# toposware/certificate-stark

Measured on NVIDIA B200. Metric: state_transition_prove_throughput, higher is better.
Workload: dtype u64 (f63 modular)

## Files before the change

### certificate_stark_b200/csrc/airs.cuh

```cuda
#pragma once
#include "ecc.cuh"
#include "rescue.cuh"
#include "rescue_tables.h"
#include <stdexcept>

#if defined(__CUDA_ARCH__)
#define CSG_PRAGMA_(x) _Pragma(#x)
#define CSG_PRAGMA(x) CSG_PRAGMA_(x)
#else
#define CSG_PRAGMA(x)
#endif
#ifndef CSG_REST_UNROLL
#define CSG_REST_UNROLL 1
#endif
#if defined(__CUDA_ARCH__)
#define CSG_REST_LOOP CSG_PRAGMA(unroll CSG_REST_UNROLL)
#else
#define CSG_REST_LOOP
#endif
#ifndef CSG_RESCUE_FWD_UNROLL
#define CSG_RESCUE_FWD_UNROLL 2
#endif

namespace airs {
using f63::fe;

enum : int { TRANSACTION = 0, MERKLE_UPDATE = 1, MERKLE_INIT = 2, SCHNORR = 3, RANGE = 4, RESCUE = 5 };

enum : int {
    HSW = 14, HRW = 7, APW = 12, PPW = 18, PCW = 6,
    SENDER_INITIAL = 0, SENDER_BIT = 14, SENDER_UPDATED = 15, RECEIVER_INITIAL = 29, RECEIVER_BIT = 43, RECEIVER_UPDATED = 44,
    PREV_ROOT = 58, VALUE_RES = 65, BALANCE_RES = 90, NONCE_RES = 91, INT_ROOT_RES = 92, ROOT_MATCH_RES = 99,
    SENDER_KEY = 65, RECEIVER_KEY = 77, DELTA_COPY = 89, SIGMA_COPY = 90, NONCE_COPY = 91,
    SENDER_KEY_RES = 101, RECEIVER_KEY_RES = 103, DELTA_COPY_RES = 105, SIGMA_COPY_RES = 106, NONCE_COPY_RES = 107,
    DELTA_RANGE_RES = 108, SIGMA_RANGE_RES = 109,
    DELTA_BIT = 56, DELTA_ACC = 57, SIGMA_BIT = 92, SIGMA_ACC = 93,
    LIMBS = 2 * PPW + 1,
    SIG_HASH = 2 * PPW + 6
};
enum : int {
    TX_SETUP = 0, TX_MERKLE = 1, TX_HASH_INPUT = 2, TX_FINISH = 3, TX_HASH = 4, TX_SCHNORR = 5, TX_SCALAR_MULT = 6, TX_DOUBLING = 7,
    TX_DIGEST = 8, TX_SCHNORR_HASH = 12, TX_INTERNAL = 13, TX_RANGE_STEP = 17, TX_RANGE_FINISH = 18, TX_VALUE_COPY = 19, TX_ARK = 20
};

constexpr int MAX_GROUPS = 8;

struct Frame {
    const fe *cur_p, *next_p;
    size_t stride;
    CSG_HD fe cur(int c) const { return cur_p[(size_t)c * stride]; }
    CSG_HD fe next(int c) const { return next_p[(size_t)c * stride]; }
};
struct Periodic {
    const fe *tab;
    const uint32_t *off, *mask;
    uint32_t i;
    CSG_HD fe operator()(int c) const { return tab[off[c] + (i & mask[c])]; }
};

#if defined(__CUDACC__)
static __host__ __device__ __noinline__
#else
inline
#endif
fe slot_coefficient(const fe *alpha, const fe *beta, const uint8_t *group, const fe *xp, size_t xp_stride, int slot) {
    return f63::add(alpha[slot], f63::mul(beta[slot], xp[group[slot] * xp_stride]));
}

constexpr int MAX_SPLIT_GROUPS = 6;
template <bool SPLIT, int DEG = 1>
struct CombT {
    static constexpr bool split = SPLIT;
    static constexpr int D = DEG;

    const fe *alpha, *beta;
    const uint8_t *group;
    const fe *xp;
    size_t xp_stride;
// ... 95 lines not shown

CSG_HD fe f_not(fe a) { return f63::sub(f63::ONE, a); }
CSG_HD fe f_bin(fe a) { return f63::sub(f63::sqr(a), a); }

template <class PV, class CB>
CSG_HD void rescue_state(const Frame &f, const PV &pv, CB &C, int col0, int ark0, fe flag_a, int slot_a, bool second, fe flag_b, int slot_b) {
    fe tc[14], tn[14];
#if defined(__CUDA_ARCH__)
#pragma unroll
#endif
    for (int j = 0; j < 14; j++) {
        tc[j] = rescue::cube(f.cur(col0 + j));
        tn[j] = f63::sub(f.next(col0 + j), pv(ark0 + 14 + j));
    }
    FlagAcc a(flag_a), b(flag_b);
#if defined(__CUDA_ARCH__)
#pragma unroll 1
#endif
    for (int i = 0; i < 14; i++) {
        const uint64_t *mds = CSG_TABLE(CSG_MDS) + i * 14, *inv_mds = CSG_TABLE(CSG_INV_MDS) + i * 14;
        f63::acc128 fwd, bwd;
#if defined(__CUDA_ARCH__)
#pragma unroll
#endif
        for (int j = 0; j < 14; j++) { fwd.mac(mds[j], tc[j]); bwd.mac(inv_mds[j], tn[j]); }
        const fe d = f63::sub(rescue::cube(bwd.reduce()), f63::add(fwd.reduce(), pv(ark0 + i)));
        a.add(C, slot_a + i, d);
        if (second) b.add(C, slot_b + i, d);
    }
    a.flush(C);
    if (second) b.flush(C);
}

template <class CB>
CSG_HD void merkle_auth_path(const Frame &f, CB &C, int base, fe tx_hash, fe hash_input, fe hashf) {
    const fe copy_flag = f63::mul(tx_hash, f_not(f63::add(hashf, hash_input)));
    const fe init_flag = f63::mul(tx_hash, hash_input);
    const fe bit = f.next(base + HSW), nbit = f_not(bit);
    C.add(base + HSW, f63::mul(tx_hash, f_bin(bit)));
    const fe init_bit = f63::mul(init_flag, bit), init_nbit = f63::mul(init_flag, nbit);
    FlagAcc keep(f63::add(copy_flag, init_nbit)), to_rate(init_bit), place_bit(init_bit), place_nbit(init_nbit);
#if defined(__CUDA_ARCH__)
#pragma unroll 1
#endif
    for (int k = 0; k < 2; k++) {
        const int o = base + k * (HSW + 1);
        CSG_REST_LOOP
        for (int i = 0; i < HRW; i++) {
            fe c = f.cur(o + i);
            keep.add(C, o + i, f63::sub(c, f.next(o + i)));
            to_rate.add(C, o + HRW + i, f63::sub(c, f.next(o + HRW + i)));
        }
        C.sync();
    }
    CSG_REST_LOOP
    for (int i = 0; i < HRW; i++) place_bit.add(C, base + i, f63::sub(f.next(base + HSW + 1 + i), f.next(base + i)));
    CSG_REST_LOOP
    for (int i = HRW; i < HSW; i++) place_nbit.add(C, base + i, f63::sub(f.next(base + HSW + 1 + i), f.next(base + i)));
    C.sync();
    keep.flush(C);
    to_rate.flush(C);
    place_bit.flush(C);
    place_nbit.flush(C);
}
template <class CB>
CSG_HD void merkle_roots(const Frame &f, CB &C, fe finish) {
    FlagAcc carry(f_not(finish)), fin(finish);
    CSG_REST_LOOP
    for (int i = 0; i < HRW; i++) {
        fe nr = f.next(PREV_ROOT + i), cr = f.cur(PREV_ROOT + i);
        carry.add(C, PREV_ROOT + i, f63::sub(nr, cr));
        fin.add(C, PREV_ROOT + i, f63::sub(nr, f.next(RECEIVER_UPDATED + i)));
        fin.add(C, INT_ROOT_RES + i, f63::sub(f.cur(SENDER_UPDATED + i), f.cur(RECEIVER_INITIAL + i)));
        fin.add(C, ROOT_MATCH_RES + i, f63::sub(f.next(SENDER_INITIAL + i), cr));
    }
    carry.flush(C);
    fin.flush(C);
}
template <class CB>
CSG_HD void value_block(const Frame &f, CB &C, FlagAcc &a) {
    CSG_REST_LOOP
    for (int i = 0; i < APW; i++) {
        a.add(C, VALUE_RES + i, f63::sub(f.cur(SENDER_INITIAL + i), f.cur(SENDER_UPDATED + i)));
        a.add(C, VALUE_RES + APW + i, f63::sub(f.cur(RECEIVER_INITIAL + i), f.cur(RECEIVER_UPDATED + i)));
    }
    a.add(C, VALUE_RES + 2 * APW, f63::sub(f.cur(RECEIVER_INITIAL + APW + 1), f.cur(RECEIVER_UPDATED + APW + 1)));
    a.add(C, BALANCE_RES, f63::sub(f63::sub(f.cur(SENDER_INITIAL + APW), f.cur(SENDER_UPDATED + APW)),
                                   f63::sub(f.cur(RECEIVER_UPDATED + APW), f.cur(RECEIVER_INITIAL + APW))));
    a.add(C, NONCE_RES, f63::sub(f.cur(SENDER_UPDATED + APW + 1), f63::add(f.cur(SENDER_INITIAL + APW + 1), f63::ONE)));
}

template <class CB>
CSG_HD void scalar_mult_bank(const Frame &f, CB &C, int o, const fe (&q)[12], fe doubling, fe addition) {
    auto load_point = [&]() {
        ecc::point p;
#if defined(__CUDA_ARCH__)
#pragma unroll
#endif
        for (int i = 0; i < 6; i++) { p.x.c[i] = f.cur(o + i); p.y.c[i] = f.cur(o + 6 + i); p.z.c[i] = f.cur(o + 12 + i); }
        return p;
    };
    const fe bit = f.cur(o + PPW);
    {
        ecc::point d = ecc::double_point(load_point());
        FlagAcc a(doubling);
        for (int i = 0; i < 6; i++) {
            a.add(C, o + i, f63::sub(f.next(o + i), d.x.c[i]));
            a.add(C, o + 6 + i, f63::sub(f.next(o + 6 + i), d.y.c[i]));
            a.add(C, o + 12 + i, f63::sub(f.next(o + 12 + i), d.z.c[i]));
        }
        a.add(C, o + PPW, f_bin(bit));
        a.flush(C);
    }
// ... 8 lines not shown
        }
        a.add(C, o + PPW, f63::sub(bit, f.next(o + PPW)));
        a.flush(C);
    }
}
template <class CB>
CSG_HD void scalar_mult_bank_outputs(const Frame &f, CB &C, int o, const fe (&q)[12], int formula) {
    ecc::point p;
#if defined(__CUDA_ARCH__)
#pragma unroll
#endif
    for (int i = 0; i < 6; i++) { p.x.c[i] = f.cur(o + i); p.y.c[i] = f.cur(o + 6 + i); p.z.c[i] = f.cur(o + 12 + i); }
    const ecc::point r = formula == 0 ? ecc::double_point(p) : ecc::add_mixed(p, ecc::load6(q), ecc::load6(q + 6));
    FlagAcc a(f63::ONE);
    for (int i = 0; i < 6; i++) a.add(C, o + i, r.x.c[i]);
    for (int i = 0; i < 6; i++) a.add(C, o + 6 + i, r.y.c[i]);
    for (int i = 0; i < 6; i++) a.add(C, o + 12 + i, r.z.c[i]);
    a.flush(C);
}
template <class CB>
CSG_HD fe scalar_mult_bank_merge(const Frame &f, const CB &C, int comp, int o, fe doubling, fe addition, fe Cd, fe Cm) {
    const fe bit = f.cur(o + PPW), nbit = f_not(bit);
    f63::acc192 sd, sa;
    for (int i = 0; i < PPW; i++) {
        const fe c = comp ? C.coef_x(comp, o + i) : C.coef(o + i), nx = f.next(o + i);
        sd.mac(c, nx);
        sa.mac(c, f63::sub(nx, f63::mul(nbit, f.cur(o + i))));
    }
    const fe cb = comp ? C.coef_x(comp, o + PPW) : C.coef(o + PPW);
    const fe td = f63::sub(f63::add(sd.reduce(), f63::mul(cb, f_bin(bit))), Cd);
    const fe ta = f63::sub(f63::add(sa.reduce(), f63::mul(cb, f63::sub(bit, f.next(o + PPW)))), f63::mul(bit, Cm));
    return f63::add(f63::mul(doubling, td), f63::mul(addition, ta));
}
template <class CB>
CSG_HD void schnorr_final_addition(const Frame &f, CB &C, fe final_add) {
    ecc::point s, hp;
    for (int i = 0; i < 6; i++) {
        s.x.c[i] = f.cur(i); s.y.c[i] = f.cur(6 + i); s.z.c[i] = f.cur(12 + i);
        hp.x.c[i] = f.cur(PPW + 1 + i); hp.y.c[i] = f.cur(PPW + 7 + i); hp.z.c[i] = f.cur(PPW + 13 + i);
    }
    ecc::point r = ecc::add_full(s, hp);
    ecc::fp6 nx;
    for (int i = 0; i < 6; i++) nx.c[i] = f.next(i);
    ecc::fp6 xz = ecc::mul(nx, r.z);
    FlagAcc a(final_add);
    for (int i = 0; i < 6; i++) {
        a.add(C, i, f63::sub(xz.c[i], r.x.c[i]));
        a.add(C, 6 + i, f63::sub(f.next(6 + i), r.y.c[i]));
        a.add(C, 12 + i, f63::sub(f.next(12 + i), r.z.c[i]));
    }
    for (int i = 0; i < 4; i++) a.add(C, LIMBS + 1 + i, f63::sub(f.cur(LIMBS + 1 + i), f.cur(SIG_HASH + i)));
    a.flush(C);
}
template <class IN, class CB>
CSG_HD void schnorr_light(const Frame &f, CB &C, fe doubling, fe addition, const fe (&digest)[4], fe copy_hash, IN in) {
    const fe hbit_next = f.next(LIMBS);
    FlagAcc hold(addition);
    CSG_REST_LOOP
    for (int i = 0; i < 4; i++) {
        const int c = LIMBS + 4 - i;
        fe cv = f.cur(c), nv = f.next(c);
        C.add(c, f63::mul(f63::mul(digest[i], doubling), f63::sub(nv, f63::add(f63::dbl(cv), hbit_next))));
        C.add(c, f63::mul(f63::mul(f_not(digest[i]), doubling), f63::sub(cv, nv)));
        hold.add(C, LIMBS + 1 + i, f63::sub(f.cur(LIMBS + 1 + i), f.next(LIMBS + 1 + i)));
    }
    hold.flush(C);
    C.sync();
    FlagAcc a(copy_hash);
    CSG_REST_LOOP
    for (int i = 0; i < HRW; i++) {
        a.add(C, SIG_HASH + i, f63::sub(f.cur(SIG_HASH + i), f.next(SIG_HASH + i)));
        a.add(C, SIG_HASH + HRW + i, f63::sub(f.next(SIG_HASH + HRW + i), in(i)));
    }
    a.flush(C);
}

template <int AIR> struct Items;
template <> struct Items<TRANSACTION> { static constexpr int rescue = 5, ecc = 3; };
template <> struct Items<MERKLE_UPDATE> { static constexpr int rescue = 4, ecc = 0; };
template <> struct Items<MERKLE_INIT> { static constexpr int rescue = 4, ecc = 0; };
template <> struct Items<SCHNORR> { static constexpr int rescue = 1, ecc = 3; };
template <> struct Items<RANGE> { static constexpr int rescue = 0, ecc = 0; };
template <> struct Items<RESCUE> { static constexpr int rescue = 1, ecc = 0; };

struct RescueItem { int col0, ark0, slot_a, slot_b; bool second; };
CSG_HD constexpr RescueItem rescue_item(int air, int s) {
    return air == TRANSACTION ? (s < 4 ? RescueItem{15 * s - (s >> 1), TX_ARK, 14 * s, 15 * s - (s >> 1), true} : RescueItem{SIG_HASH, TX_ARK, SIG_HASH, 0, false})
         : air == MERKLE_UPDATE ? RescueItem{15 * s - (s >> 1), 5, 15 * s - (s >> 1), 0, false}
// ... 111 lines not shown
            else if (s == 2) rescue_state_t<rescue_item_ng(TRANSACTION, 2, 0), rescue_item_ng(TRANSACTION, 2, 1)>(f, pv, C, it.col0, it.ark0, flag_a, 4, flag_b, 5);
            else if (s == 3) rescue_state_t<rescue_item_ng(TRANSACTION, 3, 0), rescue_item_ng(TRANSACTION, 3, 1)>(f, pv, C, it.col0, it.ark0, flag_a, 6, flag_b, 7);
            else rescue_state_t<rescue_item_ng(TRANSACTION, 4, 0), 0>(f, pv, C, it.col0, it.ark0, flag_a, 8, 0, 0);
        } else rescue_state_t<1, 0>(f, pv, C, it.col0, it.ark0, flag_a, 2 * s, 0, 0);
        return;
    }
    rescue_state(f, pv, C, it.col0, it.ark0, flag_a, it.slot_a, it.second, flag_b, it.slot_b);
}
template <int AIR, class PV, class CB>
CSG_HD void eval_ecc_bank(int bank, const Frame &f, const PV &pv, CB &C) {
    if (AIR != TRANSACTION && AIR != SCHNORR) return;
    const fe scalar_mult = pv(AIR == TRANSACTION ? TX_SCALAR_MULT : 1);
    const fe doubling = pv(AIR == TRANSACTION ? TX_DOUBLING : 2), addition = f63::mul(f_not(doubling), scalar_mult);
    fe q[12];
    const uint64_t *gen = CSG_TABLE(CSG_GENERATOR);
    for (int j = 0; j < 12; j++) q[j] = bank == 0 ? gen[j] : (AIR == TRANSACTION ? f.next(SENDER_KEY + j) : pv(7 + j));
    scalar_mult_bank(f, C, bank * (PPW + 1), q, doubling, addition);
}
template <int AIR, class PV, class CB>
CSG_HD void eval_ecc_bank_outputs(int bank, int formula, const Frame &f, const PV &pv, CB &C) {
    if (AIR != TRANSACTION && AIR != SCHNORR) return;
    fe q[12];
    const uint64_t *gen = CSG_TABLE(CSG_GENERATOR);
    for (int j = 0; j < 12; j++) q[j] = bank == 0 ? gen[j] : (AIR == TRANSACTION ? f.next(SENDER_KEY + j) : pv(7 + j));
    scalar_mult_bank_outputs(f, C, bank * (PPW + 1), q, formula);
}
template <int AIR, class PV, class CB>
CSG_HD fe eval_ecc_bank_merge(int bank, const Frame &f, const PV &pv, const CB &C, int comp, fe Cd, fe Cm) {
    if (AIR != TRANSACTION && AIR != SCHNORR) return 0;
    const fe scalar_mult = pv(AIR == TRANSACTION ? TX_SCALAR_MULT : 1);
    const fe doubling = pv(AIR == TRANSACTION ? TX_DOUBLING : 2), addition = f63::mul(f_not(doubling), scalar_mult);
    return scalar_mult_bank_merge(f, C, comp, bank * (PPW + 1), doubling, addition, Cd, Cm);
}
template <int AIR, class PV, class CB>
CSG_HD void eval_ecc_final(const Frame &f, const PV &pv, CB &C) {
    if (AIR != TRANSACTION && AIR != SCHNORR) return;
    const fe mask = pv(AIR == TRANSACTION ? TX_SCHNORR : 0), scalar_mult = pv(AIR == TRANSACTION ? TX_SCALAR_MULT : 1);
    schnorr_final_addition(f, C, f63::mul(f_not(scalar_mult), mask));
}

template <class PV, class CB>
CSG_HD void rest_transaction(const Frame &f, const PV &pv, CB &C) {
    const fe setup = pv(TX_SETUP), tx_hash = pv(TX_MERKLE), hash_input = pv(TX_HASH_INPUT), finish = pv(TX_FINISH), hashf = pv(TX_HASH);
    const fe schnorr_mask = pv(TX_SCHNORR), scalar_mult = pv(TX_SCALAR_MULT), doubling = pv(TX_DOUBLING), schnorr_hash = pv(TX_SCHNORR_HASH);
    const fe copy_hash = f63::mul(f_not(schnorr_hash), schnorr_mask);
    const fe addition = f63::mul(f_not(doubling), scalar_mult);
    {
        FlagAcc a(setup);
        value_block(f, C, a);
        C.sync();
        CSG_REST_LOOP
        for (int o = 0; o < APW; o++) {
            a.add(C, SENDER_KEY_RES + o, f63::sub(f.next(SENDER_KEY + o), f.cur(SENDER_INITIAL + o)));
            a.add(C, RECEIVER_KEY_RES + o, f63::sub(f.next(RECEIVER_KEY + o), f.cur(RECEIVER_INITIAL + o)));
        }
        a.add(C, DELTA_COPY_RES, f63::sub(f.next(DELTA_COPY), f63::sub(f.cur(SENDER_INITIAL + APW), f.cur(SENDER_UPDATED + APW))));
        a.add(C, SIGMA_COPY_RES, f63::sub(f.next(SIGMA_COPY), f.cur(SENDER_UPDATED + APW)));
        a.add(C, NONCE_COPY_RES, f63::sub(f.next(NONCE_COPY), f.cur(SENDER_INITIAL + APW + 1)));
        a.flush(C);
    }
    C.sync();
    {
        FlagAcc a(pv(TX_VALUE_COPY));
        CSG_REST_LOOP
        for (int o = 0; o < APW; o++) {
            a.add(C, SENDER_KEY_RES + o, f63::sub(f.next(SENDER_KEY + o), f.cur(SENDER_KEY + o)));
            a.add(C, RECEIVER_KEY_RES + o, f63::sub(f.next(RECEIVER_KEY + o), f.cur(RECEIVER_KEY + o)));
        }
        a.add(C, DELTA_COPY_RES, f63::sub(f.next(DELTA_COPY), f.cur(DELTA_COPY)));
        a.add(C, SIGMA_COPY_RES, f63::sub(f.next(SIGMA_COPY), f.cur(SIGMA_COPY)));
        a.add(C, NONCE_COPY_RES, f63::sub(f.next(NONCE_COPY), f.cur(NONCE_COPY)));
        a.flush(C);
    }
    C.sync();
#if defined(__CUDA_ARCH__)
// ... 5 lines not shown

    const fe k0 = pv(TX_INTERNAL), k1 = pv(TX_INTERNAL + 1), k2 = pv(TX_INTERNAL + 2), k3 = pv(TX_INTERNAL + 3);
    auto cell = [&](int idx) -> fe {
        if (idx < 2 * APW) return f.next(SENDER_KEY + idx);
        if (idx == 2 * APW) return f.next(DELTA_COPY);
        if (idx == 2 * APW + 1) return f.next(NONCE_COPY);
        return 0;
    };
    auto in = [&](int i) -> fe {
        f63::acc128 t;
        t.mac(k0, cell(i)); t.mac(k1, cell(HRW + i)); t.mac(k2, cell(2 * HRW + i)); t.mac(k3, cell(3 * HRW + i));
        return t.reduce();
    };
    const fe digest[4] = {pv(TX_DIGEST), pv(TX_DIGEST + 1), pv(TX_DIGEST + 2), pv(TX_DIGEST + 3)};
    schnorr_light(f, C, doubling, addition, digest, copy_hash, in);
    C.sync();

    {
        FlagAcc a(pv(TX_RANGE_STEP));
        fe db = f.next(DELTA_BIT), sb = f.next(SIGMA_BIT);
        a.add(C, DELTA_ACC, f63::sub(f.next(DELTA_ACC), f63::add(f63::dbl(f.cur(DELTA_ACC)), db)));
        a.add(C, DELTA_BIT, f_bin(db));
        a.add(C, SIGMA_ACC, f63::sub(f.next(SIGMA_ACC), f63::add(f63::dbl(f.cur(SIGMA_ACC)), sb)));
        a.add(C, SIGMA_BIT, f_bin(sb));
        a.flush(C);
        FlagAcc b(pv(TX_RANGE_FINISH));
        fe v = f63::sub(f.next(DELTA_ACC), f.next(DELTA_COPY));
        b.add(C, DELTA_RANGE_RES, v);
        b.add(C, SIGMA_RANGE_RES, v);
        b.flush(C);
    }
}

template <int AIR, class PV, class CB>
CSG_HD void eval_rest(const Frame &f, const PV &pv, CB &C) {
    if (AIR == TRANSACTION) rest_transaction(f, pv, C);
    else if (AIR == MERKLE_UPDATE) {
        FlagAcc a(pv(0));
        value_block(f, C, a);
        a.flush(C);
#if defined(__CUDA_ARCH__)
#pragma unroll 1
#endif
        for (int path = 0; path < 2; path++) merkle_auth_path(f, C, path == 0 ? SENDER_INITIAL : RECEIVER_INITIAL, pv(1), pv(2), pv(4));
        merkle_roots(f, C, pv(3));
    } else if (AIR == SCHNORR) {
        const fe global = pv(0), scalar_mult = pv(1), doubling = pv(2), hash_flag = pv(APW + 7);
        const fe digest[4] = {pv(3), pv(4), pv(5), pv(6)};
        schnorr_light(f, C, doubling, f63::mul(f_not(doubling), scalar_mult), digest, f63::mul(f_not(hash_flag), global), [&](int i) { return pv(APW + 8 + i); });
    } else if (AIR == RANGE) {
        fe b = f.next(0);
        C.add(1, f63::sub(f.next(1), f63::add(f63::dbl(f.cur(1)), b)));
        C.add(0, f_bin(b));
    } else if (AIR == RESCUE) {
        FlagAcc a(f_not(pv(0)));
        for (int i = 0; i < HRW; i++) {
            a.add(C, i, f63::sub(f.cur(i), f.next(i)));
            a.add(C, HRW + i, f.next(HRW + i));
        }
        a.flush(C);
    }
}

template <int AIR, class PV, class CB>
CSG_HD void eval_transition(const Frame &f, const PV &pv, CB &C) {
    for (int s = 0; s < Items<AIR>::rescue; s++) eval_rescue_item<AIR>(s, f, pv, C);
    if (Items<AIR>::ecc) { eval_ecc_bank<AIR>(0, f, pv, C); eval_ecc_bank<AIR>(1, f, pv, C); eval_ecc_final<AIR>(f, pv, C); }
    eval_rest<AIR>(f, pv, C);
// ... 4 lines not shown
```

### certificate_stark_b200/csrc/constraints_kernels.cuh

```cuda
#pragma once
#include <cstdlib>
#include <vector>

#include "airs.cuh"
#include "constraints.cuh"
#include "stages.cuh"

namespace csg {
using namespace f63;

namespace {
constexpr int CONS_THREADS = 128;

struct RowCtx {
    airs::Frame f;
    airs::Periodic pv;
    fe x;
};
__device__ __forceinline__ void prefetch_tile_l2(const fe *base, unsigned long long col_stride, unsigned col0, unsigned ncols, unsigned long long i0,
                                                 unsigned long long n) {
#ifndef CSG_NO_TILE_PREFETCH
    const unsigned long long rows = n - i0 < (unsigned long long)CONS_THREADS + 2 ? n - i0 : (unsigned long long)CONS_THREADS + 2;
    const unsigned bytes = (unsigned)(rows * sizeof(fe)) & ~15u;
    if (!bytes) return;
    for (unsigned c = threadIdx.x; c < ncols; c += CONS_THREADS)
        asm volatile("cp.async.bulk.prefetch.L2.global [%0], %1;" ::"l"(base + (unsigned long long)(col0 + c) * col_stride + i0), "r"(bytes) : "memory");
#endif
}

__device__ __forceinline__ RowCtx row_setup(const ConsArgs *__restrict__ A, const fe *__restrict__ lde, const fe *__restrict__ W,
                                            const fe *__restrict__ ptab, unsigned kc, unsigned long long i, fe (*xp_s)[CONS_THREADS]) {
    const unsigned long long n = 1ULL << A->logn, inext = (i + 1) & (n - 1);
    const fe *base = lde + A->lde_coset_stride[kc];
    RowCtx r{airs::Frame{base + i, base + inext, (size_t)A->col_stride},
             airs::Periodic{ptab + kc * A->ptab_coset_stride, A->poff, A->pmask, (uint32_t)i}, mul(A->shift[kc], W[i])};
    for (unsigned g = 0; g < A->ngroups; g++) xp_s[g][threadIdx.x] = mul(A->shift_adj[kc][g], W[(A->adj_mod[g] * i) & (n - 1)]);
    return r;
}

constexpr int INV_CHUNK = 16, INV_THREADS = 128;
__global__ void __launch_bounds__(INV_THREADS) boundary_inverse_kernel(const ConsArgs *__restrict__ A, const fe *__restrict__ W, fe *__restrict__ binv) {
    const unsigned kc = blockIdx.y, g = blockIdx.z;
    const unsigned long long n = 1ULL << A->logn;
    const unsigned long long base = blockIdx.x * (unsigned long long)(INV_CHUNK * INV_THREADS) + threadIdx.x;
    const fe shift = A->b_steps[g] == 1 ? A->shift[kc] : A->b_shift_steps[kc][g], off = A->b_offset[g];
// ... 13 lines not shown
        const unsigned long long i = base + (unsigned long long)c * INV_THREADS;
        if (i < n) out[i] = mul(ainv, pre[c]);
        ainv = mul(ainv, d[c]);
    }
}

#ifndef CSG_ECC_MINBLOCKS
#define CSG_ECC_MINBLOCKS 3
#endif
#ifndef CSG_RESCUE_MINBLOCKS
#define CSG_RESCUE_MINBLOCKS 6
#endif
#ifndef CSG_LOW_MINBLOCKS
#define CSG_LOW_MINBLOCKS 4
#endif
#ifndef CSG_REST_MINBLOCKS
#define CSG_REST_MINBLOCKS 6
#endif
template <int AIR, int KIND, int DEG = 1>
__global__ void __launch_bounds__(CONS_THREADS, KIND == 0 ? (DEG == 1 && AIR != airs::TRANSACTION ? CSG_RESCUE_MINBLOCKS : 4) : CSG_ECC_MINBLOCKS)
cons_item_kernel(const ConsArgs *__restrict__ A, const fe *__restrict__ lde, const fe *__restrict__ W, const fe *__restrict__ ptab,
                 fe *__restrict__ part, unsigned part_items) {
    __shared__ fe xp_s[airs::MAX_GROUPS][CONS_THREADS];
    const unsigned kc = blockIdx.y, item = KIND == 2 ? 2 : blockIdx.z;
    const unsigned long long n = 1ULL << A->logn, i = blockIdx.x * (unsigned long long)CONS_THREADS + threadIdx.x;
    if (i >= n) return;
    RowCtx r = row_setup(A, lde, W, ptab, kc, i, xp_s);
    airs::CombT<false, DEG> C{A->alpha, A->beta, A->group, &xp_s[0][threadIdx.x], (size_t)CONS_THREADS, acc192(), nullptr, 0,
                              &A->alpha_x[0][0], &A->beta_x[0][0], (size_t)CONS_MAX_CONSTRAINTS};
    C.rt = &A->rt;
    if (KIND == 0) airs::eval_rescue_item<AIR>((int)item, r.f, r.pv, C);
    else if (KIND == 1) airs::eval_ecc_bank<AIR>((int)item, r.f, r.pv, C);
    else airs::eval_ecc_final<AIR>(r.f, r.pv, C);
    part[((unsigned long long)item * A->ncosets + kc) * n + i] = C.sum.reduce();
#pragma unroll
    for (int j = 1; j < DEG; j++) part[(((unsigned long long)j * part_items + item) * A->ncosets + kc) * n + i] = C.sum_x[j - 1].reduce();
}

template <int AIR, int DEG = 1>
__global__ void __launch_bounds__(CONS_THREADS, DEG == 1 ? CSG_REST_MINBLOCKS : 4)
cons_rest_kernel(const ConsArgs *__restrict__ A, const fe *__restrict__ lde, const fe *__restrict__ W, const fe *__restrict__ ptab,
                 const fe *__restrict__ apoly, const fe *__restrict__ part, unsigned nparts, const fe *__restrict__ binv, fe *__restrict__ out) {
    __shared__ fe xp_s[airs::MAX_GROUPS][CONS_THREADS];
    const unsigned kc = blockIdx.y;
    const unsigned long long n = 1ULL << A->logn, i = blockIdx.x * (unsigned long long)CONS_THREADS + threadIdx.x;
    if (i >= n) return;
    RowCtx r = row_setup(A, lde, W, ptab, kc, i, xp_s);
    airs::CombT<false, DEG> C{A->alpha, A->beta, A->group, &xp_s[0][threadIdx.x], (size_t)CONS_THREADS, acc192(), nullptr, 0,
                              &A->alpha_x[0][0], &A->beta_x[0][0], (size_t)CONS_MAX_CONSTRAINTS};
    airs::eval_rest<AIR>(r.f, r.pv, C);
    const fe x = r.x;
    fe res[DEG];
#pragma unroll
    for (int j = 0; j < DEG; j++) {
        fe t = j == 0 ? C.sum.reduce() : C.sum_x[j > 0 ? j - 1 : 0].reduce();
        for (unsigned p = 0; p < nparts; p++) t = add(t, part[(((unsigned long long)j * nparts + p) * A->ncosets + kc) * n + i]);
        res[j] = mul(mul(t, sub(x, A->g_last)), A->zinv[kc]);
    }
    unsigned a = 0;
    for (unsigned g = 0; g < A->nbgroups; g++) {
        const fe xpb = mul(A->b_shift_adj[kc][g], W[(A->b_adj_mod[g] * i) & (n - 1)]);
        acc192 s[DEG];
        for (; a < A->nassertions && A->a_group[a] == g; a++) {
            fe v = A->a_value[a];
            if (A->a_poly_len[a] > 1) {
                const fe *poly = apoly + A->a_poly_off[a];
// ... 11 lines not shown
        for (int j = 0; j < DEG; j++) res[j] = add(res[j], mul(s[j].reduce(), bi));
    }
#pragma unroll
    for (int j = 0; j < DEG; j++) out[((unsigned long long)j * A->ncosets + kc) * n + i] = res[j];
}

template <int AIR, int DEG = 1>
void launch(const ConsArgs *args_dev, const ConsArgs &h, const fe *lde, const fe *W, const fe *ptab, const fe *apoly, fe *part, fe *out, Stream &st,
            cudaEvent_t *ev) {
    const unsigned long long n = 1ULL << h.logn;
    const unsigned gx = (unsigned)((n + CONS_THREADS - 1) / CONS_THREADS);
    constexpr int NR = airs::Items<AIR>::rescue, NE = airs::Items<AIR>::ecc;
    auto mark = [&](int k) { if (ev) CSG_CUDA(cudaEventRecord(ev[k], st.s)); };
    mark(0);
    if (NR > 0) CSG_LAUNCH(st, (cons_item_kernel<AIR, 0, DEG>), dim3(gx, h.ncosets, NR > 0 ? NR : 1), CONS_THREADS, 0, args_dev, lde, W, ptab, part, (unsigned)(NR + NE));
    mark(1);
    mark(5);
    fe *ecc_part = part + (size_t)NR * h.ncosets * n;
    if (NE > 0) CSG_LAUNCH(st, (cons_item_kernel<AIR, 1, DEG>), dim3(gx, h.ncosets, 2), CONS_THREADS, 0, args_dev, lde, W, ptab, ecc_part, (unsigned)(NR + NE));
    mark(2);
    if (NE > 0) CSG_LAUNCH(st, (cons_item_kernel<AIR, 2, DEG>), dim3(gx, h.ncosets, 1), CONS_THREADS, 0, args_dev, lde, W, ptab, ecc_part, (unsigned)(NR + NE));
    mark(3);
    fe *binv = part + (size_t)DEG * (NR + NE) * h.ncosets * n;
    if (h.nbgroups > 0)
        CSG_LAUNCH(st, boundary_inverse_kernel, dim3((unsigned)((n + INV_CHUNK * INV_THREADS - 1) / (INV_CHUNK * INV_THREADS)), h.ncosets, h.nbgroups),
                   INV_THREADS, 0, args_dev, W, binv);
    CSG_LAUNCH(st, (cons_rest_kernel<AIR, DEG>), dim3(gx, h.ncosets), CONS_THREADS, 0, args_dev, lde, W, ptab, apoly, (const fe *)part, (unsigned)(NR + NE),
               (const fe *)binv, out);
    mark(4);
}

constexpr size_t split_smem_bytes(int deg) { return (size_t)3 * airs::MAX_SPLIT_GROUPS * deg * CONS_THREADS * sizeof(uint64_t); }

template <int AIR, int KIND, int DEG>
__global__ void __launch_bounds__(CONS_THREADS, CSG_LOW_MINBLOCKS)
cons_low_kernel(const ConsArgs *__restrict__ A, const fe *__restrict__ lde, const fe *__restrict__ W, const fe *__restrict__ ptab,
                fe *__restrict__ low, unsigned item0) {
    extern __shared__ uint64_t part_dyn[];
    const unsigned j = blockIdx.y, kc = 2 * j, item = item0 + blockIdx.z, L = A->ncosets / 2, NP = 1 + A->ngroups;
    const unsigned long long n = 1ULL << A->logn, i = blockIdx.x * (unsigned long long)CONS_THREADS + threadIdx.x;
    if (i >= n) return;
    const unsigned long long inext = (i + 1) & (n - 1);
    const fe *base = lde + A->lde_coset_stride[kc];
    if (KIND == 3) prefetch_tile_l2(base, A->col_stride, 0, A->width, blockIdx.x * (unsigned long long)CONS_THREADS, n);
    airs::Frame f{base + i, base + inext, (size_t)A->col_stride};
    airs::Periodic pv{ptab + kc * A->ptab_coset_stride, A->poff, A->pmask, (uint32_t)i};
    for (unsigned k = 0; k < 3 * airs::MAX_SPLIT_GROUPS * DEG; k++) part_dyn[k * CONS_THREADS + threadIdx.x] = 0;
    airs::CombT<true, DEG> C{A->alpha, A->beta, A->group, nullptr, 0, acc192(), &part_dyn[threadIdx.x], (size_t)CONS_THREADS,
                             &A->alpha_x[0][0], &A->beta_x[0][0], (size_t)CONS_MAX_CONSTRAINTS};
    C.rt = &A->rt;
    if (KIND == 0) airs::eval_rescue_item<AIR>((int)blockIdx.z, f, pv, C);
    else airs::eval_rest<AIR>(f, pv, C);
#pragma unroll
    for (int comp = 0; comp < DEG; comp++) {
        fe *dst = low + ((((unsigned long long)item * DEG + comp) * NP) * L + j) * n + i;
        dst[0] = comp == 0 ? C.sum.reduce() : C.sum_x[comp > 0 ? comp - 1 : 0].reduce();
        for (unsigned g = 0; g + 1 < NP; g++) dst[(unsigned long long)(1 + g) * L * n] = C.part_value((int)g, comp);
    }
}

constexpr unsigned ECC_SPLIT_MAX_POLYS = 16;
constexpr unsigned ECC_SUPER = 512;
struct EccSplitMap {
    unsigned npolys[2];
    unsigned char groups[2][airs::MAX_SPLIT_GROUPS];
    unsigned base[4];
    unsigned total;
};
template <int AIR, int DEG>
__global__ void __launch_bounds__(CONS_THREADS, CSG_ECC_MINBLOCKS)
cons_ecc_low_kernel(const ConsArgs *__restrict__ A, const fe *__restrict__ lde, const fe *__restrict__ ptab, EccSplitMap M, fe *__restrict__ eccl) {
    extern __shared__ uint64_t part_dyn[];
    const unsigned j = blockIdx.y, kc = 2 * j, L = A->ncosets / 2;
    const unsigned rem = blockIdx.x % (4 * ECC_SUPER), v = rem / ECC_SUPER, bank = v >> 1, npb = M.npolys[bank];
    const unsigned long long n = 1ULL << A->logn, tile = (unsigned long long)(blockIdx.x / (4 * ECC_SUPER)) * ECC_SUPER + rem % ECC_SUPER;
    const unsigned long long i = tile * CONS_THREADS + threadIdx.x;
    if (i >= n) return;
    const unsigned long long inext = (i + 1) & (n - 1);
    const fe *base = lde + A->lde_coset_stride[kc];
    airs::Frame f{base + i, base + inext, (size_t)A->col_stride};
    airs::Periodic pv{ptab + kc * A->ptab_coset_stride, A->poff, A->pmask, (uint32_t)i};
    for (unsigned k = 0; k < 3 * airs::MAX_SPLIT_GROUPS * DEG; k++) part_dyn[k * CONS_THREADS + threadIdx.x] = 0;
    airs::CombT<true, DEG> C{A->alpha, A->beta, A->group, nullptr, 0, acc192(), &part_dyn[threadIdx.x], (size_t)CONS_THREADS,
                             &A->alpha_x[0][0], &A->beta_x[0][0], (size_t)CONS_MAX_CONSTRAINTS};
    airs::eval_ecc_bank_outputs<AIR>((int)bank, (int)(v & 1), f, pv, C);
#pragma unroll
    for (int comp = 0; comp < DEG; comp++) {
        fe *dst = eccl + (((unsigned long long)M.base[v] * DEG + comp * npb) * L + j) * n + i;
        dst[0] = comp == 0 ? C.sum.reduce() : C.sum_x[comp > 0 ? comp - 1 : 0].reduce();
        for (unsigned q = 0; q + 1 < npb; q++) dst[(unsigned long long)(1 + q) * L * n] = C.part_value((int)M.groups[bank][q], comp);
    }
}
// ... 136 lines not shown
            for (unsigned q = 0; q < cnt; q++) seen = seen || M.groups[b][q] == h.group[sl];
            if (!seen) M.groups[b][cnt++] = h.group[sl];
        }
        M.npolys[b] = 1 + cnt;
    }
    for (unsigned v = 0; v < 4; v++) { M.base[v] = M.total; M.total += M.npolys[v >> 1]; }
    if (M.total > ECC_SPLIT_MAX_POLYS) throw std::runtime_error("too many degree groups for the curve split");
    const size_t eslab = (size_t)DEG * M.total * L * n;
    fe *eccl_even = binv + (size_t)CONS_MAX_BGROUPS * ce * n, *eccl_coef = eccl_even + eslab, *eccl_mix = eccl_coef + eslab, *eccl_odd = eccl_mix + eslab;
    const size_t smem = split_smem_bytes(DEG);
    if (smem > 48 * 1024) {
        CSG_CUDA(cudaFuncSetAttribute((cons_low_kernel<AIR, 0, DEG>), cudaFuncAttributeMaxDynamicSharedMemorySize, (int)smem));
        CSG_CUDA(cudaFuncSetAttribute((cons_low_kernel<AIR, 3, DEG>), cudaFuncAttributeMaxDynamicSharedMemorySize, (int)smem));
        CSG_CUDA(cudaFuncSetAttribute((cons_ecc_low_kernel<AIR, DEG>), cudaFuncAttributeMaxDynamicSharedMemorySize, (int)smem));
    }
    auto mark = [&](int k) { if (ev) CSG_CUDA(cudaEventRecord(ev[k], st.s)); };
    host_mark("  cons: split setup");
    mark(0);
    CSG_LAUNCH(st, (cons_low_kernel<AIR, 0, DEG>), dim3(gx, L, NR), CONS_THREADS, smem, args_dev, lde, W, ptab, low_parts, 0u);
    mark(1);
    if (ecc_split) {
        CSG_LAUNCH(st, (cons_ecc_low_kernel<AIR, DEG>), dim3((gx + ECC_SUPER - 1) / ECC_SUPER * 4 * ECC_SUPER, L, 1), CONS_THREADS, smem, args_dev, lde, ptab, M, eccl_even);
        mark(5);
        host_mark("  cons: low + curve-low launched");
        extend(eccl_even, eccl_coef, eccl_mix, eccl_odd, DEG * M.total);
        host_mark("  cons: curve polynomials extended");
        CSG_LAUNCH(st, (cons_ecc_merge_kernel<AIR, DEG>), dim3(gx, ce, 2), CONS_THREADS, 0, args_dev, lde, W, ptab, M, (const fe *)eccl_even, (const fe *)eccl_odd, hi,
                   (unsigned)NE);
    } else {
        mark(5);
        CSG_LAUNCH(st, (cons_item_kernel<AIR, 1, DEG>), dim3(gx, ce, 2), CONS_THREADS, 0, args_dev, lde, W, ptab, hi, (unsigned)NE);
    }
    mark(2);
    CSG_LAUNCH(st, (cons_item_kernel<AIR, 2, DEG>), dim3(gx, ce, 1), CONS_THREADS, 0, args_dev, lde, W, ptab, hi, (unsigned)NE);
    mark(3);
    CSG_LAUNCH(st, (cons_low_kernel<AIR, 3, DEG>), dim3(gx, L, 1), CONS_THREADS, smem, args_dev, lde, W, ptab, low_parts, (unsigned)NR);
    sum_slices(low_parts, low_sum, slab, NR + 1, st);
    host_mark("  cons: merge, final item, rest launched");
    extend(low_sum, low_coef, low_mix, low_odd, NPD);
    host_mark("  cons: low polynomials extended");
    if (h.nbgroups > 0)
        CSG_LAUNCH(st, boundary_inverse_kernel, dim3((unsigned)((n + INV_CHUNK * INV_THREADS - 1) / (INV_CHUNK * INV_THREADS)), ce, h.nbgroups),
                   INV_THREADS, 0, args_dev, W, binv);
    CSG_LAUNCH(st, cons_final_kernel<DEG>, dim3(gx, ce), CONS_THREADS, 0, args_dev, lde, W, apoly, (const fe *)low_sum, (const fe *)low_odd, (const fe *)hi,
               (unsigned)NE, (const fe *)binv, out);
    mark(4);
}

}
}
```

Baseline: 17390.

## Load LDE row tiles into shared memory via TMA for final-add and rest kernels

Adds a row-tile loader that uses a TMA tensor map and an mbarrier to bulk-copy a block's 128 rows across all needed columns into shared memory, plus a small edge row for the next-row wrap. The Schnorr final-add kernel and the rest-constraint kernel (DEG==1) now read cur/next values from shared memory instead of strided global loads. Constraint helpers are templated on the frame type so they work with both frames. The cost is more dynamic shared memory per block, which can lower occupancy, plus host-side tensor-map encoding on every launch.

```diff
diff --git a/certificate_stark_b200/csrc/airs.cuh b/certificate_stark_b200/csrc/airs.cuh
--- a/certificate_stark_b200/csrc/airs.cuh
+++ b/certificate_stark_b200/csrc/airs.cuh
@@ -44,6 +44,7 @@
 };
 
 constexpr int MAX_GROUPS = 8;
+constexpr int FINAL_ADD_COLS = SIG_HASH + 4;
 
 struct Frame {
     const fe *cur_p, *next_p;
@@ -205,8 +206,8 @@
     if (second) b.flush(C);
 }
 
-template <class CB>
-CSG_HD void merkle_auth_path(const Frame &f, CB &C, int base, fe tx_hash, fe hash_input, fe hashf) {
+template <class FR, class CB>
+CSG_HD void merkle_auth_path(const FR &f, CB &C, int base, fe tx_hash, fe hash_input, fe hashf) {
     const fe copy_flag = f63::mul(tx_hash, f_not(f63::add(hashf, hash_input)));
     const fe init_flag = f63::mul(tx_hash, hash_input);
     const fe bit = f.next(base + HSW), nbit = f_not(bit);
@@ -236,8 +237,8 @@
     place_bit.flush(C);
     place_nbit.flush(C);
 }
-template <class CB>
-CSG_HD void merkle_roots(const Frame &f, CB &C, fe finish) {
+template <class FR, class CB>
+CSG_HD void merkle_roots(const FR &f, CB &C, fe finish) {
     FlagAcc carry(f_not(finish)), fin(finish);
     CSG_REST_LOOP
     for (int i = 0; i < HRW; i++) {
@@ -250,8 +251,8 @@
     carry.flush(C);
     fin.flush(C);
 }
-template <class CB>
-CSG_HD void value_block(const Frame &f, CB &C, FlagAcc &a) {
+template <class FR, class CB>
+CSG_HD void value_block(const FR &f, CB &C, FlagAcc &a) {
     CSG_REST_LOOP
     for (int i = 0; i < APW; i++) {
         a.add(C, VALUE_RES + i, f63::sub(f.cur(SENDER_INITIAL + i), f.cur(SENDER_UPDATED + i)));
@@ -326,8 +327,8 @@
     const fe ta = f63::sub(f63::add(sa.reduce(), f63::mul(cb, f63::sub(bit, f.next(o + PPW)))), f63::mul(bit, Cm));
     return f63::add(f63::mul(doubling, td), f63::mul(addition, ta));
 }
-template <class CB>
-CSG_HD void schnorr_final_addition(const Frame &f, CB &C, fe final_add) {
+template <class FR, class CB>
+CSG_HD void schnorr_final_addition(const FR &f, CB &C, fe final_add) {
     ecc::point s, hp;
     for (int i = 0; i < 6; i++) {
         s.x.c[i] = f.cur(i); s.y.c[i] = f.cur(6 + i); s.z.c[i] = f.cur(12 + i);
@@ -346,8 +347,8 @@
     for (int i = 0; i < 4; i++) a.add(C, LIMBS + 1 + i, f63::sub(f.cur(LIMBS + 1 + i), f.cur(SIG_HASH + i)));
     a.flush(C);
 }
-template <class IN, class CB>
-CSG_HD void schnorr_light(const Frame &f, CB &C, fe doubling, fe addition, const fe (&digest)[4], fe copy_hash, IN in) {
+template <class FR, class IN, class CB>
+CSG_HD void schnorr_light(const FR &f, CB &C, fe doubling, fe addition, const fe (&digest)[4], fe copy_hash, IN in) {
     const fe hbit_next = f.next(LIMBS);
     FlagAcc hold(addition);
     CSG_REST_LOOP
@@ -525,15 +526,15 @@
     const fe doubling = pv(AIR == TRANSACTION ? TX_DOUBLING : 2), addition = f63::mul(f_not(doubling), scalar_mult);
     return scalar_mult_bank_merge(f, C, comp, bank * (PPW + 1), doubling, addition, Cd, Cm);
 }
-template <int AIR, class PV, class CB>
-CSG_HD void eval_ecc_final(const Frame &f, const PV &pv, CB &C) {
+template <int AIR, class FR, class PV, class CB>
+CSG_HD void eval_ecc_final(const FR &f, const PV &pv, CB &C) {
     if (AIR != TRANSACTION && AIR != SCHNORR) return;
     const fe mask = pv(AIR == TRANSACTION ? TX_SCHNORR : 0), scalar_mult = pv(AIR == TRANSACTION ? TX_SCALAR_MULT : 1);
     schnorr_final_addition(f, C, f63::mul(f_not(scalar_mult), mask));
 }
 
-template <class PV, class CB>
-CSG_HD void rest_transaction(const Frame &f, const PV &pv, CB &C) {
+template <class FR, class PV, class CB>
+CSG_HD void rest_transaction(const FR &f, const PV &pv, CB &C) {
     const fe setup = pv(TX_SETUP), tx_hash = pv(TX_MERKLE), hash_input = pv(TX_HASH_INPUT), finish = pv(TX_FINISH), hashf = pv(TX_HASH);
     const fe schnorr_mask = pv(TX_SCHNORR), scalar_mult = pv(TX_SCALAR_MULT), doubling = pv(TX_DOUBLING), schnorr_hash = pv(TX_SCHNORR_HASH);
     const fe copy_hash = f63::mul(f_not(schnorr_hash), schnorr_mask);
@@ -605,8 +606,8 @@
     }
 }
 
-template <int AIR, class PV, class CB>
-CSG_HD void eval_rest(const Frame &f, const PV &pv, CB &C) {
+template <int AIR, class FR, class PV, class CB>
+CSG_HD void eval_rest(const FR &f, const PV &pv, CB &C) {
     if (AIR == TRANSACTION) rest_transaction(f, pv, C);
     else if (AIR == MERKLE_UPDATE) {
         FlagAcc a(pv(0));
diff --git a/certificate_stark_b200/csrc/constraints_kernels.cuh b/certificate_stark_b200/csrc/constraints_kernels.cuh
--- a/certificate_stark_b200/csrc/constraints_kernels.cuh
+++ b/certificate_stark_b200/csrc/constraints_kernels.cuh
@@ -4,6 +4,7 @@
 
 #include "airs.cuh"
 #include "constraints.cuh"
+#include "row_tile.cuh"
 #include "stages.cuh"
 
 namespace csg {
@@ -11,6 +12,7 @@
 
 namespace {
 constexpr int CONS_THREADS = 128;
+static_assert(CONS_THREADS == (int)TILE_ROWS, "a row tile holds the rows of one CTA");
 
 struct RowCtx {
     airs::Frame f;
@@ -90,6 +92,24 @@
     if (KIND == 0) airs::eval_rescue_item<AIR>((int)item, r.f, r.pv, C);
     else if (KIND == 1) airs::eval_ecc_bank<AIR>((int)item, r.f, r.pv, C);
     else airs::eval_ecc_final<AIR>(r.f, r.pv, C);
+    part[((unsigned long long)item * A->ncosets + kc) * n + i] = C.sum.reduce();
+#pragma unroll
+    for (int j = 1; j < DEG; j++) part[(((unsigned long long)j * part_items + item) * A->ncosets + kc) * n + i] = C.sum_x[j - 1].reduce();
+}
+
+template <int AIR, int DEG>
+__global__ void __launch_bounds__(CONS_THREADS, CSG_ECC_MINBLOCKS)
+cons_final_add_tile_kernel(const __grid_constant__ CUtensorMap map, const ConsArgs *__restrict__ A, const fe *__restrict__ lde, const fe *__restrict__ W,
+                           const fe *__restrict__ ptab, fe *__restrict__ part, unsigned part_items) {
+    __shared__ fe xp_s[airs::MAX_GROUPS][CONS_THREADS];
+    extern __shared__ __align__(16) unsigned char tile_dyn[];
+    const unsigned kc = blockIdx.y, item = 2;
+    const unsigned long long n = 1ULL << A->logn, i = blockIdx.x * (unsigned long long)CONS_THREADS + threadIdx.x;
+    const SmemFrame f = load_row_tile(map, A, lde, kc, 0, airs::FINAL_ADD_COLS, tile_dyn);
+    RowCtx r = row_setup(A, lde, W, ptab, kc, i, xp_s);
+    airs::CombT<false, DEG> C{A->alpha, A->beta, A->group, &xp_s[0][threadIdx.x], (size_t)CONS_THREADS, acc192(), nullptr, 0,
+                              &A->alpha_x[0][0], &A->beta_x[0][0], (size_t)CONS_MAX_CONSTRAINTS};
+    airs::eval_ecc_final<AIR>(f, r.pv, C);
     part[((unsigned long long)item * A->ncosets + kc) * n + i] = C.sum.reduce();
 #pragma unroll
     for (int j = 1; j < DEG; j++) part[(((unsigned long long)j * part_items + item) * A->ncosets + kc) * n + i] = C.sum_x[j - 1].reduce();
@@ -167,6 +187,17 @@
 
 constexpr size_t split_smem_bytes(int deg) { return (size_t)3 * airs::MAX_SPLIT_GROUPS * deg * CONS_THREADS * sizeof(uint64_t); }
 
+template <class CB>
+__device__ __forceinline__ void store_low(const CB &C, fe *__restrict__ low, unsigned item, unsigned NP, unsigned L, unsigned j, unsigned long long n,
+                                          unsigned long long i) {
+#pragma unroll
+    for (int comp = 0; comp < CB::D; comp++) {
+        fe *dst = low + ((((unsigned long long)item * CB::D + comp) * NP) * L + j) * n + i;
+        dst[0] = comp == 0 ? C.sum.reduce() : C.sum_x[comp > 0 ? comp - 1 : 0].reduce();
+        for (unsigned g = 0; g + 1 < NP; g++) dst[(unsigned long long)(1 + g) * L * n] = C.part_value((int)g, comp);
+    }
+}
+
 template <int AIR, int KIND, int DEG>
 __global__ void __launch_bounds__(CONS_THREADS, CSG_LOW_MINBLOCKS)
 cons_low_kernel(const ConsArgs *__restrict__ A, const fe *__restrict__ lde, const fe *__restrict__ W, const fe *__restrict__ ptab,
@@ -186,13 +217,25 @@
     C.rt = &A->rt;
     if (KIND == 0) airs::eval_rescue_item<AIR>((int)blockIdx.z, f, pv, C);
     else airs::eval_rest<AIR>(f, pv, C);
-#pragma unroll
-    for (int comp = 0; comp < DEG; comp++) {
-        fe *dst = low + ((((unsigned long long)item * DEG + comp) * NP) * L + j) * n + i;
-        dst[0] = comp == 0 ? C.sum.reduce() : C.sum_x[comp > 0 ? comp - 1 : 0].reduce();
-        for (unsigned g = 0; g + 1 < NP; g++) dst[(unsigned long long)(1 + g) * L * n] = C.part_value((int)g, comp);
-    }
-}
+    store_low(C, low, item, NP, L, j, n, i);
+}
+template <int AIR>
+__global__ void __launch_bounds__(CONS_THREADS, 2)
+cons_rest_tile_kernel(const __grid_constant__ CUtensorMap map, const ConsArgs *__restrict__ A, const fe *__restrict__ lde, const fe *__restrict__ ptab,
+                      fe *__restrict__ low, unsigned item) {
+    extern __shared__ __align__(16) uint64_t part_dyn[];
+    constexpr unsigned NPART = 3 * airs::MAX_SPLIT_GROUPS;
+    const unsigned j = blockIdx.y, kc = 2 * j, L = A->ncosets / 2, NP = 1 + A->ngroups;
+    const unsigned long long n = 1ULL << A->logn, i = blockIdx.x * (unsigned long long)CONS_THREADS + threadIdx.x;
+    const SmemFrame f = load_row_tile(map, A, lde, kc, 0, A->width, reinterpret_cast<unsigned char *>(part_dyn + NPART * CONS_THREADS));
+    airs::Periodic pv{ptab + kc * A->ptab_coset_stride, A->poff, A->pmask, (uint32_t)i};
+    for (unsigned k = 0; k < NPART; k++) part_dyn[k * CONS_THREADS + threadIdx.x] = 0;
+    airs::CombT<true, 1> C{A->alpha, A->beta, A->group, nullptr, 0, acc192(), &part_dyn[threadIdx.x], (size_t)CONS_THREADS,
+                           &A->alpha_x[0][0], &A->beta_x[0][0], (size_t)CONS_MAX_CONSTRAINTS};
+    airs::eval_rest<AIR>(f, pv, C);
+    store_low(C, low, item, NP, L, j, n, i);
+}
+constexpr size_t rest_tile_smem_bytes(unsigned width) { return split_smem_bytes(1) + row_tile_bytes(width); }
 
 constexpr unsigned ECC_SPLIT_MAX_POLYS = 16;
 constexpr unsigned ECC_SUPER = 512;
@@ -395,9 +438,26 @@
         CSG_LAUNCH(st, (cons_item_kernel<AIR, 1, DEG>), dim3(gx, ce, 2), CONS_THREADS, 0, args_dev, lde, W, ptab, hi, (unsigned)NE);
     }
     mark(2);
-    CSG_LAUNCH(st, (cons_item_kernel<AIR, 2, DEG>), dim3(gx, ce, 1), CONS_THREADS, 0, args_dev, lde, W, ptab, hi, (unsigned)NE);
+#ifndef CSG_NO_FINAL_TILE
+    if (n >= TILE_ROWS) {
+        const size_t fsmem = row_tile_bytes(airs::FINAL_ADD_COLS);
+        CSG_CUDA(cudaFuncSetAttribute((cons_final_add_tile_kernel<AIR, DEG>), cudaFuncAttributeMaxDynamicSharedMemorySize, (int)fsmem));
+        CSG_LAUNCH(st, (cons_final_add_tile_kernel<AIR, DEG>), dim3(gx, ce, 1), CONS_THREADS, fsmem, lde_tile_map(lde, h, airs::FINAL_ADD_COLS), args_dev, lde, W, ptab,
+                   hi, (unsigned)NE);
+    } else
+#endif
+        CSG_LAUNCH(st, (cons_item_kernel<AIR, 2, DEG>), dim3(gx, ce, 1), CONS_THREADS, 0, args_dev, lde, W, ptab, hi, (unsigned)NE);
     mark(3);
-    CSG_LAUNCH(st, (cons_low_kernel<AIR, 3, DEG>), dim3(gx, L, 1), CONS_THREADS, smem, args_dev, lde, W, ptab, low_parts, (unsigned)NR);
+    bool rest_done = false;
+#ifndef CSG_NO_REST_TILE
+    if constexpr (DEG == 1) if (n >= TILE_ROWS) {
+        const size_t rsmem = rest_tile_smem_bytes(h.width);
+        CSG_CUDA(cudaFuncSetAttribute(cons_rest_tile_kernel<AIR>, cudaFuncAttributeMaxDynamicSharedMemorySize, (int)rsmem));
+        CSG_LAUNCH(st, cons_rest_tile_kernel<AIR>, dim3(gx, L, 1), CONS_THREADS, rsmem, lde_tile_map(lde, h, h.width), args_dev, lde, ptab, low_parts, (unsigned)NR);
+        rest_done = true;
+    }
+#endif
+    if (!rest_done) CSG_LAUNCH(st, (cons_low_kernel<AIR, 3, DEG>), dim3(gx, L, 1), CONS_THREADS, smem, args_dev, lde, W, ptab, low_parts, (unsigned)NR);
     sum_slices(low_parts, low_sum, slab, NR + 1, st);
     host_mark("  cons: merge, final item, rest launched");
     extend(low_sum, low_coef, low_mix, low_odd, NPD);
diff --git a/certificate_stark_b200/csrc/row_tile.cuh b/certificate_stark_b200/csrc/row_tile.cuh
--- /dev/null
+++ b/certificate_stark_b200/csrc/row_tile.cuh
@@ -0,0 +1,71 @@
+#pragma once
+#include <algorithm>
+
+#include <cuda.h>
+#include <cudaTypedefs.h>
+
+#include "constraints.cuh"
+
+namespace csg {
+
+constexpr unsigned TILE_ROWS = 128;
+
+struct SmemFrame {
+    const fe *cur_p, *next_p;
+    unsigned next_stride;
+    CSG_HD fe cur(int c) const { return cur_p[c * TILE_ROWS]; }
+    CSG_HD fe next(int c) const { return next_p[c * next_stride]; }
+};
+constexpr size_t row_tile_bytes(unsigned ncols) { return (size_t)ncols * (TILE_ROWS + 1) * sizeof(fe) + sizeof(uint64_t); }
+
+inline CUtensorMap lde_tile_map(const fe *lde, const ConsArgs &h, unsigned ncols) {
+    static PFN_cuTensorMapEncodeTiled encode = [] {
+        void *fn = nullptr;
+        cudaDriverEntryPointQueryResult q{};
+        CSG_CUDA(cudaGetDriverEntryPoint("cuTensorMapEncodeTiled", &fn, cudaEnableDefault, &q));
+        if (q != cudaDriverEntryPointSuccess || !fn) throw std::runtime_error("cuTensorMapEncodeTiled is not available from the driver");
+        return (PFN_cuTensorMapEncodeTiled)fn;
+    }();
+    const unsigned long long n = 1ULL << h.logn;
+    unsigned long long cols = 0;
+    for (unsigned kc = 0; kc < h.ncosets; kc++) {
+        if (h.col_stride != n || h.lde_coset_stride[kc] % n) throw std::runtime_error("row tiles need an LDE laid out [column][row]");
+        cols = std::max(cols, h.lde_coset_stride[kc] / n + h.width);
+    }
+    if (ncols > h.width || ncols > 256 || (uintptr_t)lde % 16) throw std::runtime_error("row tile outside the limits of a TMA box");
+    CUtensorMap map;
+    const cuuint64_t dim[2] = {n, cols}, stride[1] = {n * sizeof(fe)};
+    const cuuint32_t box[2] = {TILE_ROWS, ncols}, estride[2] = {1, 1};
+    const CUresult r = encode(&map, CU_TENSOR_MAP_DATA_TYPE_UINT64, 2, (void *)lde, dim, stride, box, estride, CU_TENSOR_MAP_INTERLEAVE_NONE,
+                              CU_TENSOR_MAP_SWIZZLE_NONE, CU_TENSOR_MAP_L2_PROMOTION_L2_256B, CU_TENSOR_MAP_FLOAT_OOB_FILL_NONE);
+    if (r != CUDA_SUCCESS) throw std::runtime_error("cuTensorMapEncodeTiled failed for the LDE row tiles");
+    return map;
+}
+
+__device__ __forceinline__ SmemFrame load_row_tile(const CUtensorMap &map, const ConsArgs *__restrict__ A, const fe *__restrict__ lde, unsigned kc,
+                                                   unsigned col0, unsigned ncols, unsigned char *smem) {
+    fe *tile = reinterpret_cast<fe *>(smem), *edge = tile + ncols * TILE_ROWS;
+    uint64_t *bar = reinterpret_cast<uint64_t *>(edge + ncols);
+    const unsigned bar_s = (unsigned)__cvta_generic_to_shared(bar);
+    const unsigned long long n = 1ULL << A->logn, i0 = blockIdx.x * (unsigned long long)TILE_ROWS;
+    if (threadIdx.x == 0) {
+        const unsigned bytes = ncols * TILE_ROWS * (unsigned)sizeof(fe);
+        const int x = (int)i0, y = (int)(A->lde_coset_stride[kc] / n + col0);
+        asm volatile("mbarrier.init.shared::cta.b64 [%0], 1;" ::"r"(bar_s) : "memory");
+        asm volatile("fence.mbarrier_init.release.cluster;" ::: "memory");
+        asm volatile("mbarrier.arrive.expect_tx.shared::cta.b64 _, [%0], %1;" ::"r"(bar_s), "r"(bytes) : "memory");
+        asm volatile("cp.async.bulk.tensor.2d.shared::cluster.global.tile.mbarrier::complete_tx::bytes [%0], [%1, {%2, %3}], [%4];" ::"r"(
+                         (unsigned)__cvta_generic_to_shared(tile)),
+                     "l"(reinterpret_cast<unsigned long long>(&map)), "r"(x), "r"(y), "r"(bar_s)
+                     : "memory");
+    }
+    const fe *base = lde + A->lde_coset_stride[kc] + (unsigned long long)col0 * n + ((i0 + TILE_ROWS) & (n - 1));
+    for (unsigned c = threadIdx.x; c < ncols; c += blockDim.x) edge[c] = base[(unsigned long long)c * n];
+    __syncthreads();
+    for (unsigned done = 0; !done;)
+        asm volatile("{\n .reg .pred p;\n mbarrier.try_wait.parity.shared::cta.b64 p, [%1], 0;\n selp.u32 %0, 1, 0, p;\n}" : "=r"(done) : "r"(bar_s) : "memory");
+    const unsigned t = threadIdx.x;
+    return t + 1 < TILE_ROWS ? SmemFrame{tile + t, tile + t + 1, TILE_ROWS} : SmemFrame{tile + t, edge, 1};
+}
+
+}
```

After: 17420, median of 6. No clear change (+0.2%).
